# BVE-Reborn/rend3

Measured on AMD Instinct MI355X. Metric: shaded Mpixels/s @4K (whole frame: cull+compact all cameras, 4 shadow views, PBR opaque, tonemap), higher is better.
Workload: dtype f32; 1 GPU; BASELINE.json configs[2] stand-in: bistro_like (seed 0xB157, every object owns its geometry), 3840x2160, full PBR opaque + 4 directional shadow views (2048^2), camera dolly, 130 materials with base colour + normal + AO/roughness/metallic maps (RGBA8, mips, trilinear); objects=3000, triangles=2823212, cameras=5, parallelism=single GPU

## Files before the change

rend3_amd/csrc/kernels_shade.h:

```cpp
#pragma once
#include <type_traits>

#include "device_math.h"
#include "texture.h"

#define R3N_TEX_OCC 5
#define R3N_MS_OCC 4

struct TriRecord;
struct ViewLights;
struct ShadeArgs {
    const unsigned long long *vis;
    uint32_t width, height, row_begin, row_end;
    const r3n_frame_uniforms496 *fu;
    const r3n_camera_header240 *hdr;
    const r3n_object128 *objects;
    const uint32_t *mesh;
    const r3n_baked128 *baked;
    const r3n_material208 *materials;
    uint32_t n_materials;
    const uint32_t *tri_base;
    const uint32_t *slot_table;
    uint32_t slot_table_size;
    const uint8_t *dir_buf;
// ... 1049 lines not shown
    } else {
        h[0] = hdr[i0];
        h[1] = two ? hdr[i0 + 1u] : make_ushort4(0, 0, 0, 0);
    }
    uchar4 o8[2];
#pragma unroll
    for (int k = 0; k < 2; ++k) {
        o8[k] = tonemap_half4(srgb_lut, h[k], bgr);
        if (out_f32 != nullptr && (k == 0 || two)) {
            const float r = (float)__builtin_bit_cast(_Float16, h[k].x), g = (float)__builtin_bit_cast(_Float16, h[k].y);
            const float b = (float)__builtin_bit_cast(_Float16, h[k].z), al = (float)__builtin_bit_cast(_Float16, h[k].w);
            out_f32[i0 + (size_t)k] = make_float4(manual ? srgb_scene_to_display(r) : srgb_oetf(r), manual ? srgb_scene_to_display(g) : srgb_oetf(g),
                                                  manual ? srgb_scene_to_display(b) : srgb_oetf(b),
                                                  (!(al > 0.0f)) ? 0.0f : (al >= 1.0f ? 1.0f : al));
        }
    }
    out[i0] = o8[0];
    if (two) out[i0 + 1u] = o8[1];
}
#endif

extern "C" {
int r3n_internal_build_srgb_lut(unsigned char *lut, hipStream_t stream);
int r3n_internal_shade_prepass(const ShadeArgs *a, int tex, size_t first_key, size_t n_keys, hipStream_t stream);
int r3n_internal_resolve(const ShadeArgs *a, uint32_t samples, int tex, int rec, int split, int fast, hipStream_t stream);
int r3n_internal_resolve_class(const ShadeArgs *a, uint32_t variant, int fast, hipStream_t stream);
int r3n_internal_blend_apply(const ShadeArgs *a, const BlendApplyArgs *b, uint32_t samples, int tex, hipStream_t stream);
int r3n_internal_resolve_samples(const ushort4 *samples, ushort4 *hdr_out, size_t first_pixel, size_t n_pixels, hipStream_t stream);
int r3n_internal_tonemap(const ushort4 *hdr, uchar4 *out, float4 *out_f32, size_t first_pixel, size_t n_pixels, const unsigned char *srgb_lut,
                         uint32_t output_format, hipStream_t stream);
}
```

rend3_amd/csrc/r3n.hip:

```cpp
#include <fcntl.h>
#include <hip/hip_runtime.h>
#include <time.h>
#include <unistd.h>

#include <algorithm>
#include <atomic>
#include <cstdio>
#include <cstdlib>
#include <cstring>
#include <map>
#include <string>
#include <vector>

#include "comm.h"
#include "kernels_cull.h"
#include "kernels_raster.h"
#define R3N_SHADE_DECL_ONLY
#include "kernels_shade.h"
#include "skybox.h"
#include "blend_sort.h"
#include "morph.h"

namespace {

// ... 43 lines not shown
#define R3N_QLANES R3N_AUX_STREAMS
static_assert(R3N_AUX_STREAMS >= 1, "the shadow views draw on auxiliary streams");

struct r3n_ctx {
    int device = 0;
    hipStream_t stream = nullptr;
    hipStream_t aux[R3N_AUX_STREAMS] = {};
    hipEvent_t fork_ev[R3N_AUX_STREAMS] = {};
    hipStream_t shade = nullptr;
    hipEvent_t vp_ev = nullptr, shade_done[2] = {nullptr, nullptr};
    bool shade_pending[2] = {false, false};
    bool shade_unjoined = false;
    int shade_last = 0;
    int slot = 0;
    uint64_t frame_no = 0;
    bool overlap = true;
    bool always_fork = false;
    bool resolve_classes = true;
    bool fused_frame = false;
    DevBuf alt_vis, alt_atlas, alt_vp_baked;
    static constexpr size_t kFbUniforms = 0, kFbViewportHdr = 512, kFbDir = 768, kFbShadowHdr = 3072,
                            kFbPoint = kFbShadowHdr + 256 * R3N_MAX_SHADOW_VIEWS, kFbBytes = kFbPoint + 8448;
    static constexpr int kFbHost = 4;
    DevBuf fb_dev[2];
    uint8_t *fb_host[kFbHost] = {};
    hipEvent_t fb_ev[kFbHost] = {};
    bool fb_pending[kFbHost] = {};
    uint64_t main_epoch = 1, lane_epoch[R3N_AUX_STREAMS] = {};
    DevBuf big_count_all;
    std::vector<uint8_t> h_dir, h_point;
    uint64_t lights_version = 1, slot_lights_version[2] = {0, 0};
    hipEvent_t join_ev[R3N_AUX_STREAMS] = {};
    bool aux_used[R3N_AUX_STREAMS] = {};
    bool multi_stream = true;
    std::string err;
    DevBuf mesh, objects, materials, material_keys, dir_buf, point_buf, fu;
    DevBuf spheres, obj_meta;
    bool meta_dirty = false;
    uint32_t capacity = 0, n_materials = 0;
    std::vector<uint32_t> h_ntri;
    std::vector<uint32_t> h_material;
    std::vector<uint8_t> h_material_key;
    std::vector<r3n_material208> h_materials;
    std::vector<uint8_t> h_tex_short;
    DevBuf material_feat;
    DevBuf view_lights[2];
    uint32_t resolve_variants = 0;
    bool classes_dirty = true;
    struct Tune {
        uint32_t big_lds = R3N_BIG_LDS, vp_big_lds = R3N_VIEWPORT_BIG_LDS;
        uint32_t small_lds = R3N_SMALL_LDS, vp_small_lds = 0;
        uint32_t cut_big_lds = 0, vp_cut_big_lds = 0, cut_small_lds = 0, vp_cut_small_lds = 0;
        uint32_t prio_main = 1, prio_shade = 1, prio_aux = 1;
        uint32_t timed_pipeline = 0;
// ... 3 lines not shown
        uint32_t comm_serial = 1;
    } tune;
    bool cutout_short_dirty = true, cutout_short = false;
    bool key_census_dirty = true;
    uint64_t key_objects[3] = {0, 0, 0};
    uint64_t total_tris = 0;
    bool tri_base_dirty = true;
    DevBuf tri_base, slot_table;
    DevBuf skin_inputs, skin_matrices, skin_wave_skeleton, skin_wave_first, skin_joint_counts;
    uint32_t skinning_mode = R3N_SKIN_EXACT, skin_max_joints = 0;
    std::vector<r3n_skinning_input40> h_skin_inputs;
    uint32_t skin_total_waves = 0;
    DevBuf morph_block;
    uint32_t slot_table_size = 0;
    CamState canon;
    uint32_t width = 0, height = 0, samples = 1, atlas_w = 0, atlas_h = 0;
    float clear[4] = {0, 0, 0, 0};
    bool in_frame = false;
    bool blended_this_frame = false;
    bool resolved_this_frame = false;
    DevBuf vis, hdr16, out8, out_f32, atlas, hiz;
    r3n_hiz_desc hizd{};
    bool hiz_plane_ready = false;
    DevBuf tri_rec, tri_seen;
    DevBuf blend_order, blend_rank_base, frag_keys, frag_vals, frag_count, frag_head, samples16;
    uint32_t *status_host = nullptr, *status_dev = nullptr;
    std::vector<uint32_t> h_blend_order;
    uint32_t n_blend = 0, blend_tris = 0;
    DevBuf blend_set_slots, blend_set_locations, blend_sort_scratch;
    bool blend_sorted = false;
    uint32_t frag_capacity = 32u << 20;
    DevBuf tex_descs, tex_texels, tex_level_off, srgb8_decode;
    uint32_t n_textures = 0;
    uint64_t n_texels = 0;
    struct Cube { size_t first_word; uint32_t n, srgb; };
    DevBuf cube_texels;
    std::vector<Cube> cubes;
    uint32_t sky_cube = 0;
    bool sky_window = false;
    bool resolve_on_shade = false;
    uint32_t sky_samples_form = R3N_SKY_SAMPLES_ALL;
    DevBuf edge_list, edge_count;
    uint32_t edge_capacity_override = 0;
    DevBuf anim_rigs, anim_joints, anim_clips, anim_tracks, anim_times, anim_values, pose_requests;
    std::vector<r3n_anim_rig16> h_anim_rigs;
    std::vector<r3n_anim_clip16> h_anim_clips;
    uint32_t n_pose_requests = 0, pose_matrix_end = 0, anim_max_joints = 1;
// ... 188 lines not shown
    }
    ~Timed() {
        if (c->sync_stages) {
            (void)hipStreamSynchronize(stream);
            crumb(c, "stage done", stage);
        }
        if (!a) return;
        (void)hipEventRecord(b, stream);
        c->spans.push_back({a, b, stage, stream});
    }
};

int cam_lane(const r3n_ctx *c, r3n_camera cam) {
    if (cam == R3N_CAMERA_VIEWPORT || !c->multi_stream) return 0;
    return 1 + (int)(cam % R3N_AUX_STREAMS);
}
hipStream_t lane_stream(const r3n_ctx *c, int lane) { return lane == 0 ? c->stream : c->aux[lane - 1]; }

int fork_lane(r3n_ctx *c, int lane) {
    if (lane == 0) return R3N_OK;
    const int k = lane - 1;
    c->aux_used[k] = true;
    if (c->lane_epoch[k] == c->main_epoch && !c->always_fork) return R3N_OK;
    HIP_TRY(c, hipEventRecord(c->fork_ev[k], c->stream));
    HIP_TRY(c, hipStreamWaitEvent(c->aux[k], c->fork_ev[k], 0));
    c->lane_epoch[k] = c->main_epoch;
    return R3N_OK;
}
int join_lanes(r3n_ctx *c) {
    for (int k = 0; k < R3N_AUX_STREAMS; ++k)
        if (c->aux_used[k]) {
            HIP_TRY(c, hipEventRecord(c->join_ev[k], c->aux[k]));
            HIP_TRY(c, hipStreamWaitEvent(c->stream, c->join_ev[k], 0));
            c->aux_used[k] = false;
        }
    return R3N_OK;
}
int join_shade(r3n_ctx *c) {
    if (c->shade_unjoined) {
        HIP_TRY(c, hipStreamWaitEvent(c->stream, c->shade_done[c->shade_last], 0));
        c->shade_unjoined = false;
    }
    return R3N_OK;
}
int sync_all(r3n_ctx *c) {
    crumb(c, "sync_all");
    int r = join_lanes(c);
    if (r != R3N_OK) return r;
    r = join_shade(c);
// ... 304 lines not shown
        g_create_error = "host-mapped status word allocation failed";
        r3n_destroy(c);
        return nullptr;
    }
    c->status_host[0] = 0u;
    if (const char *eb = std::getenv("R3N_BREADCRUMBS")) {
        static std::atomic<int> n_ctx{0};
        const std::string path = std::string(eb) + ".pid" + std::to_string((long long)getpid()) + ".ctx" + std::to_string(n_ctx.fetch_add(1));
        c->crumb_fd = open(path.c_str(), O_CREAT | O_WRONLY | O_APPEND, 0644);
        crumb(c, "created");
    }
    if (const char *es = std::getenv("R3N_SYNC_STAGES")) c->sync_stages = es[0] == '1';
    if (const char *e1 = std::getenv("R3N_SINGLE_STREAM")) c->multi_stream = !(e1[0] == '1');
    if (const char *e2 = std::getenv("R3N_PIPELINE")) c->overlap = !(e2[0] == '0');
    if (const char *e5 = std::getenv("R3N_RESOLVE_CLASSES")) c->resolve_classes = !(e5[0] == '0');
    if (const char *e6 = std::getenv("R3N_ALWAYS_FORK")) c->always_fork = e6[0] == '1';
    if (const char *e3 = std::getenv("R3N_EDGE_CAPACITY")) c->edge_capacity_override = (uint32_t)std::strtoul(e3, nullptr, 10);
    if (const char *e7 = std::getenv("R3N_BIG_CAPACITY"))
        if (const uint32_t n = (uint32_t)std::strtoul(e7, nullptr, 10)) c->big_capacity = n;
    if (const char *e8 = std::getenv("R3N_FRAG_CAPACITY"))
        if (const uint32_t n = (uint32_t)std::strtoul(e8, nullptr, 10)) c->frag_capacity = n;
    if (hipStreamCreateWithPriority(&c->shade, hipStreamNonBlocking, (int)c->tune.prio_shade - 1) != hipSuccess ||
        hipEventCreateWithFlags(&c->vp_ev, hipEventDisableTiming) != hipSuccess ||
        hipEventCreateWithFlags(&c->shade_done[0], hipEventDisableTiming) != hipSuccess ||
        hipEventCreateWithFlags(&c->shade_done[1], hipEventDisableTiming) != hipSuccess) {
        g_create_error = "shade stream creation failed";
        r3n_destroy(c);
        return nullptr;
    }
    for (int k = 0; k < R3N_AUX_STREAMS; ++k)
        if (hipStreamCreateWithPriority(&c->aux[k], hipStreamNonBlocking, (int)c->tune.prio_aux - 1) != hipSuccess ||
            hipEventCreateWithFlags(&c->fork_ev[k], hipEventDisableTiming) != hipSuccess ||
            hipEventCreateWithFlags(&c->join_ev[k], hipEventDisableTiming) != hipSuccess) {
            g_create_error = "auxiliary stream creation failed";
            r3n_destroy(c);
            return nullptr;
        }
    {
        hipStream_t order[2 + R3N_AUX_STREAMS] = {c->stream, c->shade};
        for (int k = 0; k < R3N_AUX_STREAMS; ++k) order[2 + k] = c->aux[k];
        void *probe = nullptr;
        if (hipMalloc(&probe, 256) == hipSuccess) {
            for (hipStream_t st : order) {
                (void)hipMemsetAsync(probe, 0, 256, st);
                (void)hipStreamSynchronize(st);
            }
            (void)hipFree(probe);
        }
    }
    bool ok = ensure(c, c->srgb_lut, R3N_SRGB_LUT_SIZE, false, -1) == R3N_OK && ensure(c, c->srgb8_decode, 512 * 4, false, -1) == R3N_OK &&
              ensure(c, c->tex_descs, sizeof(r3n_texture_desc32), false, 0) == R3N_OK && ensure(c, c->tex_texels, 4, false, 0) == R3N_OK && ensure(c, c->tex_level_off, 64, false, 0) == R3N_OK &&
              ensure(c, c->material_keys, 256, false, 0) == R3N_OK && ensure(c, c->materials, sizeof(r3n_material208), false, 0) == R3N_OK;
    for (int k = 0; ok && k < 2; ++k) ok = ensure(c, c->fb_dev[k], r3n_ctx::kFbBytes, false, 0) == R3N_OK;
    for (int k = 0; ok && k < r3n_ctx::kFbHost; ++k)
        ok = hipHostMalloc((void **)&c->fb_host[k], r3n_ctx::kFbBytes, hipHostMallocDefault) == hipSuccess &&
             hipEventCreateWithFlags(&c->fb_ev[k], hipEventDisableTiming) == hipSuccess;
    if (ok) {
        for (int k = 0; k < r3n_ctx::kFbHost; ++k) std::memset(c->fb_host[k], 0, r3n_ctx::kFbBytes);
        c->fu.p = c->fb_dev[0].as<uint8_t>() + r3n_ctx::kFbUniforms; c->fu.bytes = 512;
        c->dir_buf.p = c->fb_dev[0].as<uint8_t>() + r3n_ctx::kFbDir; c->dir_buf.bytes = r3n_ctx::kFbShadowHdr - r3n_ctx::kFbDir;
        c->point_buf.p = c->fb_dev[0].as<uint8_t>() + r3n_ctx::kFbPoint; c->point_buf.bytes = 8448;
    }
    ok = ok && ensure(c, c->big_count_all, (size_t)(1 + R3N_QLANES) * 64 * R3N_BIGQ * 4, false, 0) == R3N_OK;
    for (int lane = 0; ok && lane < 1 + R3N_QLANES; ++lane) {
        c->big_count[lane].p = c->big_count_all.as<uint32_t>() + (size_t)lane * 64 * R3N_BIGQ;
        c->big_count[lane].bytes = 64 * R3N_BIGQ * 4;
        ok = ensure(c, c->big_items[lane], (size_t)c->big_capacity * R3N_BIGQ * sizeof(r3n_big_item), false, -1) == R3N_OK &&
             ensure(c, c->big_uv[lane], (size_t)c->big_capacity * R3N_BIGQ * sizeof(r3n_big_uv), false, -1) == R3N_OK;
    }
    if (ok) {
        (void)r3n_internal_build_srgb_lut(c->srgb_lut.as<unsigned char>(), c->stream);
        float decode[512];
        for (int i = 0; i < 256; ++i) {
            const float e = (float)i / 255.0f;
            decode[i] = e;
            decode[256 + i] = e > 0.04045f ? std::pow((e + 0.055f) / 1.055f, 2.4f) : e / 12.92f;
// ... 23 lines not shown
        g_create_error = c->err;
        r3n_destroy(c);
        return nullptr;
    }
    return c;
}

void r3n_destroy(r3n_ctx *c) {
    if (!c) return;
    crumb(c, "destroy");
    (void)hipSetDevice(c->device);
    (void)r3n_comm_destroy(c);
    if (c->stream) (void)hipStreamSynchronize(c->stream);
    if (c->shade) (void)hipStreamSynchronize(c->shade);
    for (int k = 0; k < R3N_AUX_STREAMS; ++k)
        if (c->aux[k]) (void)hipStreamSynchronize(c->aux[k]);
    for (int lane = 0; lane < 1 + R3N_QLANES; ++lane)
        for (DevBuf *b : {&c->big_items[lane], &c->big_uv[lane]})
            if (b->p) (void)hipFree(b->p);
    for (int k = 0; k < r3n_ctx::kFbHost; ++k) {
        if (c->fb_host[k]) (void)hipHostFree(c->fb_host[k]);
        if (c->fb_ev[k]) (void)hipEventDestroy(c->fb_ev[k]);
    }
    DevBuf *bufs[] = {&c->mesh, &c->objects, &c->spheres, &c->obj_meta, &c->materials, &c->material_keys, &c->fb_dev[0], &c->fb_dev[1], &c->big_count_all, &c->owners,
                      &c->tri_base, &c->slot_table, &c->skin_inputs, &c->skin_matrices, &c->skin_wave_skeleton,
                      &c->skin_wave_first, &c->skin_joint_counts, &c->morph_block, &c->vis, &c->hdr16, &c->out8, &c->out_f32, &c->atlas, &c->hiz, &c->alt_vis, &c->alt_atlas, &c->alt_vp_baked, &c->srgb_lut, &c->srgb_thr, &c->tex_descs, &c->tex_texels, &c->tex_level_off, &c->srgb8_decode,
                      &c->tri_rec, &c->tri_seen, &c->blend_order, &c->blend_rank_base, &c->frag_keys, &c->frag_vals, &c->frag_head,
                      &c->frag_count, &c->samples16, &c->anim_rigs, &c->anim_joints, &c->anim_clips, &c->anim_tracks,
                      &c->anim_times, &c->anim_values, &c->pose_requests, &c->edge_list, &c->edge_count, &c->material_feat, &c->view_lights[0],
                      &c->view_lights[1], &c->cube_texels, &c->blend_set_slots, &c->blend_set_locations, &c->blend_sort_scratch};
    for (DevBuf *b : bufs)
        if (b->p) (void)hipFree(b->p);
    free_cam(c->canon);
    free_cam(c->viewport);
    for (auto &kv : c->shadows) free_cam(kv.second);
    if (c->vp_ev) (void)hipEventDestroy(c->vp_ev);
    for (auto e : c->shade_done)
        if (e) (void)hipEventDestroy(e);
    if (c->shade) (void)hipStreamDestroy(c->shade);
    for (auto &s : c->spans) { (void)hipEventDestroy(s.a); (void)hipEventDestroy(s.b); }
    for (auto e : c->event_pool) (void)hipEventDestroy(e);
    for (int k = 0; k < R3N_AUX_STREAMS; ++k) {
        if (c->fork_ev[k]) (void)hipEventDestroy(c->fork_ev[k]);
        if (c->join_ev[k]) (void)hipEventDestroy(c->join_ev[k]);
        if (c->aux[k]) (void)hipStreamDestroy(c->aux[k]);
    }
    if (c->stage) (void)hipHostFree(c->stage);
    if (c->status_host) (void)hipHostFree(c->status_host);
    for (auto &b : c->bulk) {
        if (b.p) (void)hipHostFree(b.p);
        if (b.ev) (void)hipEventDestroy(b.ev);
    }
    for (auto e : c->stage_half_done)
        if (e) (void)hipEventDestroy(e);
    if (c->stream) (void)hipStreamDestroy(c->stream);
    delete c;
}

const char *r3n_last_error(const r3n_ctx *c) { return c ? c->err.c_str() : g_create_error.c_str(); }
// ... 286 lines not shown
    };
    const std::vector<uint8_t> old_dir = c->h_dir, old_point = c->h_point;
    TRY(take(c->h_dir, dir, dir_bytes, 128, R3N_MAX_DIR_LIGHTS));
    TRY(take(c->h_point, point, point_bytes, 32, R3N_MAX_POINT_LIGHTS));
    if (old_dir != c->h_dir || old_point != c->h_point) ++c->lights_version;
    return R3N_OK;
}

static int frame_begin_impl(r3n_ctx *c, const r3n_frame_uniforms496 *u, uint32_t w, uint32_t h, uint32_t samples,
                            const float clear_color[4], uint32_t atlas_w, uint32_t atlas_h, const r3n_frame_desc *d) {
    if (!c || !u || !clear_color || !w || !h) return fail(c, R3N_ERR_INVALID_ARG, "frame_begin: bad args");
    if (samples != 1 && samples != 4) return fail(c, R3N_ERR_INVALID_ARG, "frame_begin: samples must be 1 or 4 (SampleCount::One | Four)");
    if (w > 65535 || h > 65535) return fail(c, R3N_ERR_UNSUPPORTED, "frame_begin: target larger than 65535");
    if ((uint64_t)w * h * samples >= (1ull << 29) || (uint64_t)atlas_w * atlas_h >= (1ull << 30) || atlas_w > 65535 || atlas_h > 65535)
        return fail(c, R3N_ERR_UNSUPPORTED, "frame_begin: target of 2^29 samples or more / shadow atlas of 2^30 texels or more");
    HIP_TRY(c, hipSetDevice(c->device));
    c->width = w; c->height = h; c->samples = samples; c->atlas_w = atlas_w; c->atlas_h = atlas_h;
    std::memcpy(c->clear, clear_color, 16);
    const int hs = (int)(c->frame_no % (uint64_t)r3n_ctx::kFbHost);
    c->slot = (int)(c->frame_no++ & 1u);
    std::swap(c->vis, c->alt_vis);
    std::swap(c->atlas, c->alt_atlas);
    std::swap(c->viewport.baked, c->alt_vp_baked);
    uint8_t *dev = c->fb_dev[c->slot].as<uint8_t>();
    c->fu.p = dev + r3n_ctx::kFbUniforms;
    c->dir_buf.p = dev + r3n_ctx::kFbDir;
    c->point_buf.p = dev + r3n_ctx::kFbPoint;
    c->viewport.d_hdr.p = dev + r3n_ctx::kFbViewportHdr; c->viewport.d_hdr.bytes = 256;
    for (auto &kv : c->shadows) { kv.second.d_hdr.p = dev + r3n_ctx::kFbShadowHdr + 256u * (size_t)kv.first; kv.second.d_hdr.bytes = 256; }
    if (c->shade_pending[c->slot]) {
        HIP_TRY(c, hipStreamWaitEvent(c->stream, c->shade_done[c->slot], 0));
        c->shade_pending[c->slot] = false;
    }
    if (c->fb_pending[hs]) {
        HIP_WAIT(c, hipEventSynchronize(c->fb_ev[hs]));
        c->fb_pending[hs] = false;
    }
    uint8_t *host = c->fb_host[hs];
    std::memcpy(host + r3n_ctx::kFbUniforms, u, sizeof *u);
    if (c->h_dir.size() < 16) c->h_dir.assign(16, 0);
    if (c->h_point.size() < 16) c->h_point.assign(16, 0);
    std::memcpy(host + r3n_ctx::kFbDir, c->h_dir.data(), c->h_dir.size());
    size_t upto = r3n_ctx::kFbShadowHdr;
    if (d) {
        std::memcpy(host + r3n_ctx::kFbViewportHdr, d->viewport_header, sizeof(r3n_camera_header240));
        for (uint32_t v = 0; v < d->n_shadow_views; ++v)
            std::memcpy(host + r3n_ctx::kFbShadowHdr + 256u * (size_t)v, &d->shadow_views[v].header, sizeof(r3n_camera_header240));
        upto += 256u * (size_t)d->n_shadow_views;
    }
    HIP_TRY(c, hipMemcpyAsync(dev, host, upto, hipMemcpyHostToDevice, c->stream));
    if (c->slot_lights_version[c->slot] != c->lights_version) {
        std::memcpy(host + r3n_ctx::kFbPoint, c->h_point.data(), c->h_point.size());
        HIP_TRY(c, hipMemcpyAsync(dev + r3n_ctx::kFbPoint, host + r3n_ctx::kFbPoint, c->h_point.size(), hipMemcpyHostToDevice, c->stream));
        c->slot_lights_version[c->slot] = c->lights_version;
    }
    HIP_TRY(c, hipEventRecord(c->fb_ev[hs], c->stream));
    c->fb_pending[hs] = true;
    const size_t npix = (size_t)w * h;
    TRY(ensure(c, c->vis, npix * samples * 8, false, -1));
    TRY(ensure(c, c->hdr16, npix * 8, false, -1));
    TRY(ensure(c, c->out8, npix * 4, false, -1));
    build_hiz_desc(c->hizd, w, h);
    TRY(ensure(c, c->hiz, hiz_elements(c->hizd) * 4, false, -1));
    const size_t apix = (size_t)std::max(1u, atlas_w) * std::max(1u, atlas_h);
    TRY(ensure(c, c->atlas, apix * 4, false, -1));
    {
        Timed t(c, R3N_STAGE_CLEAR);
        hipLaunchKernelGGL(k_frame_clear, dim3(2048), dim3(256), 0, c->stream, c->vis.as<uint32_t>(), npix * samples * 2, c->atlas.as<uint32_t>(), apix,
                           c->big_count_all.as<uint32_t>(), c->big_count_all.bytes / 4);
        TRY(check_launch(c, "k_frame_clear"));
    }
    ++c->main_epoch;
    TRY(refresh_obj_meta(c));
    TRY(refresh_tri_base(c));
    c->in_frame = true;
    for (auto &f : c->forward_index_lane) f = 0;
    c->resolved_this_frame = false;
    c->blended_this_frame = false;
    c->sky_window = false;
    c->hiz_plane_ready = false;
    c->viewport.culled = false;
    for (auto &kv : c->shadows) kv.second.culled = false;
    return R3N_OK;
}

int r3n_frame_begin(r3n_ctx *c, const r3n_frame_uniforms496 *u, uint32_t w, uint32_t h, uint32_t samples,
                    const float clear_color[4], uint32_t atlas_w, uint32_t atlas_h) {
    return frame_begin_impl(c, u, w, h, samples, clear_color, atlas_w, atlas_h, nullptr);
}

int r3n_skinning(r3n_ctx *c, const r3n_skinning_input40 *inputs, uint32_t n, const float *joint_matrices, uint32_t n_joints) {
    if (!c) return R3N_ERR_INVALID_ARG;
    if (n == 0) return R3N_OK;
    if (!inputs || n_joints == 0) return fail(c, R3N_ERR_INVALID_ARG, "skinning: null inputs");
    if (!joint_matrices && c->n_pose_requests == 0) return fail(c, R3N_ERR_INVALID_ARG, "skinning: no joint matrices and no queued poses");
// ... 225 lines not shown
    TRY(ensure(c, c->pose_requests, std::max<size_t>(n, 1) * sizeof *requests, false, -1));
    if (n) {
        TRY(upload_bulk(c, c->pose_requests.p, requests, (size_t)n * sizeof *requests));
    }
    c->n_pose_requests = n;
    c->pose_matrix_end = end;
    return R3N_OK;
}


int r3n_uniform_bake(r3n_ctx *c, r3n_camera cam, const r3n_camera_header240 *hdr) {
    if (!c || !hdr) return fail(c, R3N_ERR_INVALID_ARG, "uniform_bake: null");
    CamState *s = find_cam(c, cam, true);
    if (!s) return fail(c, R3N_ERR_INVALID_ARG, "uniform_bake: bad camera");
    if (hdr->object_count != c->capacity) return fail(c, R3N_ERR_INVALID_ARG, "uniform_bake: header.object_count != object capacity");
    if ((cam == R3N_CAMERA_VIEWPORT) != (hdr->shadow_index == R3N_INVALID) || (cam != R3N_CAMERA_VIEWPORT && hdr->shadow_index != cam))
        return fail(c, R3N_ERR_INVALID_ARG, "uniform_bake: header.shadow_index does not match camera");
    HIP_TRY(c, hipSetDevice(c->device));
    s->hdr = *hdr;
    s->has_hdr = true;
    s->baked_frame = c->frame_no;
    if (c->capacity == 0) return R3N_OK;
    TRY(refresh_obj_meta(c));
    s->d_hdr.p = c->fb_dev[c->slot].as<uint8_t>() + (cam == R3N_CAMERA_VIEWPORT ? r3n_ctx::kFbViewportHdr : r3n_ctx::kFbShadowHdr + 256u * (size_t)cam);
    s->d_hdr.bytes = 256;
    if (s->hdr_frame != c->frame_no) TRY(upload_small(c, s->d_hdr.p, hdr, sizeof *hdr));
    TRY(ensure(c, s->baked, (size_t)c->capacity * sizeof(r3n_baked128), true, 0));
    const int lane = cam_lane(c, cam);
    if (c->fused_frame && c->in_frame && chained_pass_fits(c)) {
        TRY(ensure(c, s->chain, (size_t)R3N_CHAINED_OBJECT_PASS_MAX_BLOCKS * sizeof(ObjChainRec), false, 0));
        TRY(ensure(c, s->vis_flags, c->capacity, true, 0));
        TRY(ensure(c, s->vis_list, (size_t)(c->capacity + 1u) * sizeof(r3n_vis_entry), false, -1));
        TRY(ensure(c, s->slot_base[s->cur], (size_t)c->capacity * 4u, true, 0xFF));
        TRY(ensure(c, s->sub_counts[s->cur], sizeof(r3n_sub_counts), false, 0));
        TRY(ensure(c, s->counts[s->cur], sizeof(r3n_cull_counts), false, 0));
        TRY(ensure(c, s->first_entry, first_entry_bytes(c), false, -1));
        TRY(fork_lane(c, lane));
        TRY(run_bake_and_object_pass(c, *s, s->cur, camera_own(c, *s), lane_stream(c, lane), cam == R3N_CAMERA_VIEWPORT));
        s->object_pass_frame = c->frame_no;
        return R3N_OK;
    }
    TRY(fork_lane(c, lane));
    hipStream_t stream = lane_stream(c, lane);
    Timed t(c, R3N_STAGE_BAKE, stream);
    const uint32_t threads = c->capacity * 4u;
    hipLaunchKernelGGL(k_uniform_bake, dim3((threads + 255u) / 256u), dim3(256), 0, stream,
                       s->d_hdr.as<r3n_camera_header240>(), c->objects.as<r3n_object128>(), s->baked.as<r3n_baked128>());
    return check_launch(c, "k_uniform_bake");
}

static void key_census(r3n_ctx *c) {
    if (!c->key_census_dirty) return;
    c->key_objects[0] = c->key_objects[1] = c->key_objects[2] = 0;
    for (uint32_t o = 0; o < c->capacity; ++o)
        if (c->h_ntri[o]) {
            const uint32_t mi = c->h_material[o];
            c->key_objects[mi < c->h_material_key.size() ? std::min<uint32_t>(c->h_material_key[mi], 2) : 0]++;
        }
    c->key_census_dirty = false;
}
// ... 12 lines not shown
    for (int k = 0; k < 3; ++k) s->key_objects[cur][k] = c->key_objects[k];
    const int lane = cam_lane(c, cam);
    hipStream_t stream = lane_stream(c, lane);
    {
        const uint32_t cap0 = c->capacity, nblocks0 = (cap0 + 255u) / 256u;
        TRY(ensure(c, s->vis_flags, cap0, true, 0));
        TRY(ensure(c, s->vis_list, (size_t)(cap0 + 1u) * sizeof(r3n_vis_entry), false, -1));
        TRY(ensure(c, s->block_sums, (size_t)nblocks0 * sizeof(ObjBlockSums), false, -1));
        TRY(ensure(c, s->block_off, (size_t)nblocks0 * sizeof(ObjBlockOffsets), false, -1));
        TRY(ensure(c, s->slot_base[cur], (size_t)cap0 * 4u, true, 0xFF));
        if (viewport && s->has_prev) TRY(ensure(c, s->slot_base[prev], (size_t)cap0 * 4u, true, 0xFF));
        TRY(ensure(c, s->sub_counts[cur], sizeof(r3n_sub_counts), false, 0));
        TRY(ensure(c, s->counts[cur], sizeof(r3n_cull_counts), false, 0));
        TRY(ensure(c, s->first_entry, first_entry_bytes(c), false, -1));
    }
    const uint32_t mw = max_waves(c);
    const uint32_t chunks = (mw + R3N_CHUNK_WAVES - 1u) / R3N_CHUNK_WAVES;
    const uint32_t subcap = ((chunks + R3N_SUBQ - 1u) / R3N_SUBQ) * (R3N_CHUNK_WAVES * 64u);
    const size_t list_bytes = (size_t)3 * R3N_SUBQ * subcap * sizeof(r3n_tri_ref);
    s->subcap[cur] = subcap;
    TRY(ensure(c, s->mask[cur], (size_t)mw * 8u, false, -1));
    TRY(ensure(c, s->predicted[cur], list_bytes, false, -1));
    if (viewport) TRY(ensure(c, s->residual, list_bytes, false, -1));
    TRY(fork_lane(c, lane));
    if (s->object_pass_frame != c->frame_no)
        TRY(run_object_pass(c, *s, cur, camera_own(c, *s), nullptr, stream));
    TriCullArgs a{};
    a.hdr = s->d_hdr.as<r3n_camera_header240>();
    a.objects = c->objects.as<r3n_object128>();
    a.mesh = c->mesh.as<uint32_t>();
    a.baked = s->baked.as<r3n_baked128>();
    a.material_keys = c->material_keys.as<uint8_t>();
    a.n_materials = c->n_materials;
    a.vis_list = s->vis_list.as<r3n_vis_entry>();
    a.first_entry = s->first_entry.as<uint32_t>();
    a.counts = s->counts[cur].as<r3n_cull_counts>();
    a.prev_slot_base = (viewport && s->has_prev) ? s->slot_base[prev].as<uint32_t>() : nullptr;
    a.prev_mask = (viewport && s->has_prev) ? s->mask[prev].as<unsigned long long>() : nullptr;
    a.mask = s->mask[cur].as<unsigned long long>();
    a.predicted = s->predicted[cur].as<r3n_tri_ref>();
    a.residual = viewport ? s->residual.as<r3n_tri_ref>() : nullptr;
    a.sub_counts = s->sub_counts[cur].as<r3n_sub_counts>();
    a.subcap = subcap;
    a.hiz.data = c->hiz.as<float>();
    a.hiz.d = c->hizd;
    const uint32_t grid = std::max(1u, std::min(chunks, 4096u));
    {
        Timed t(c, R3N_STAGE_TRIANGLE_CULL, stream);
        hipLaunchKernelGGL(k_triangle_cull, dim3(grid), dim3(256), viewport ? c->tune.vp_cull_lds : c->tune.cull_lds, stream, a);
// ... 218 lines not shown
    a.material_feat = nullptr;
    a.variants = 0u;
    return a;
}

int r3n_resolve_opaque(r3n_ctx *c) {
    if (!c || !c->in_frame) return fail(c, R3N_ERR_STATE, "resolve_opaque: outside a frame");
    HIP_TRY(c, hipSetDevice(c->device));
    const uint32_t r0 = std::min(c->row_begin, c->height), r1 = std::min(c->row_end, c->height);
    c->sky_window = r1 <= r0;
    c->resolve_on_shade = false;
    if (r1 <= r0) return R3N_OK;
    CamState &s = c->viewport;
    if (!s.has_hdr && c->capacity) return fail(c, R3N_ERR_STATE, "resolve_opaque: viewport uniforms not baked");
    const bool use_records = c->total_tris > 0 && (uint64_t)c->total_tris * sizeof(TriRecord) <= (8ull << 30);
    const uint64_t npix_all = (uint64_t)c->width * c->height;
    const bool blend_samples = c->samples == 4 && c->blend_tris > 0;
    const bool split = c->samples == 4 && use_records && !blend_samples && npix_all < (1ull << 29);
    uint32_t edge_cap = 0;
    const bool classes = use_records && c->samples == 1 && c->n_textures > 0 && c->n_materials > 0 && c->resolve_classes;
    if (classes) TRY(refresh_material_classes(c));
    if (use_records && c->samples == 1) TRY(ensure(c, c->view_lights[c->slot], sizeof(ViewLights), false, -1));
    if (use_records) {
        TRY(ensure(c, c->tri_rec, (size_t)c->total_tris * sizeof(TriRecord), false, -1));
        TRY(ensure(c, c->tri_seen, (size_t)c->total_tris, false, 0));
    }
    const bool sky = c->sky_cube != 0u;
    const bool sky_samples = sky && c->samples == 4 && !split && !blend_samples;
    if (blend_samples || split || sky_samples) TRY(ensure(c, c->samples16, (size_t)npix_all * 4 * 8, false, -1));
    if (split) {
        edge_cap = (uint32_t)((uint64_t)(r1 - r0) * c->width * 3u / R3N_EDGEQ) + 4096u;
        if (c->edge_capacity_override) edge_cap = c->edge_capacity_override;
        TRY(ensure(c, c->edge_list, (size_t)edge_cap * R3N_EDGEQ * 4, false, -1));
        TRY(ensure(c, c->edge_count, R3N_EDGEQ * 4, false, 0));
    }
    const bool on_shade = c->overlap && c->multi_stream && (!c->timing || c->tune.timed_pipeline != 0u) && c->blend_tris == 0;
    hipStream_t stream = on_shade ? c->shade : c->stream;
    if (on_shade) {
        HIP_TRY(c, hipEventRecord(c->vp_ev, c->stream));
        HIP_TRY(c, hipStreamWaitEvent(c->shade, c->vp_ev, 0));
        for (int k = 0; k < R3N_AUX_STREAMS; ++k)
            if (c->aux_used[k]) {
                HIP_TRY(c, hipEventRecord(c->join_ev[k], c->aux[k]));
                HIP_TRY(c, hipStreamWaitEvent(c->shade, c->join_ev[k], 0));
            }
    } else {
        TRY(join_lanes(c));
        TRY(join_shade(c));
    }
    ShadeArgs a = make_shade_args(c, r0, r1);
    if (blend_samples || sky_samples) a.samples_out = c->samples16.as<ushort4>();
    if (use_records && c->samples == 1) a.view_lights = c->view_lights[c->slot].as<ViewLights>();
    if (classes && c->resolve_variants != 0u) {
        a.material_feat = c->material_feat.as<uint32_t>();
        a.variants = c->resolve_variants;
    }
    c->resolved_this_frame = true;
    const bool tex = c->n_textures > 0;
    if (use_records) {
        a.tri_rec = c->tri_rec.as<TriRecord>();
        a.seen = c->tri_seen.as<unsigned char>();
        Timed t(c, R3N_STAGE_VERTEX, stream);
        const size_t first = (size_t)r0 * c->width * c->samples, npx = (size_t)(r1 - r0) * c->width * c->samples;
        HIP_TRY(c, (hipError_t)r3n_internal_shade_prepass(&a, tex ? 1 : 0, first, npx, stream));
    }
    {
        Timed t(c, R3N_STAGE_SHADE, stream);
        if (split) {
            a.samples_out = c->samples16.as<ushort4>();
            a.edge_list = c->edge_list.as<uint32_t>();
            a.edge_count = c->edge_count.as<uint32_t>();
            a.edge_capacity = edge_cap;
            HIP_TRY(c, hipMemsetAsync(a.edge_count, 0, R3N_EDGEQ * 4, stream));
        }
        HIP_TRY(c, (hipError_t)r3n_internal_resolve(&a, c->samples, tex ? 1 : 0, a.tri_rec != nullptr ? 1 : 0, split ? (sky ? 2 : 1) : 0,
                                                    c->shade_mode == R3N_SHADE_FAST ? 1 : 0, stream));
    }
    TRY(check_launch(c, "k_resolve_opaque"));
    if (on_shade) {
        HIP_TRY(c, hipEventRecord(c->shade_done[c->slot], c->shade));
        c->shade_pending[c->slot] = true;
        c->shade_unjoined = true;
        c->shade_last = c->slot;
    }
    c->sky_window = true;
    c->resolve_on_shade = on_shade;
    c->sky_samples_form = split ? R3N_SKY_SAMPLES_EDGES : R3N_SKY_SAMPLES_ALL;
    return R3N_OK;
// ... 561 lines not shown
    }
    return r3n_output_work_enqueued(c);
}

int r3n_render_frame(r3n_ctx *c, const r3n_frame_desc *d) {
    if (!c || !d || d->struct_size < sizeof(r3n_frame_desc)) return fail(c, R3N_ERR_INVALID_ARG, "render_frame: bad descriptor");
    if (!d->uniforms || !d->viewport_header || (d->n_shadow_views && !d->shadow_views) || d->n_shadow_views > R3N_MAX_SHADOW_VIEWS)
        return fail(c, R3N_ERR_INVALID_ARG, "render_frame: null uniforms / headers, or too many shadow views");
    if (c->in_frame) return fail(c, R3N_ERR_STATE, "render_frame: a frame is already open");
    const bool native = c->comm.on;
    crumb(c, "render_frame", d->width, d->height);
    if (native) {
        if (d->exchange) return fail(c, R3N_ERR_INVALID_ARG, "render_frame: an exchange callback AND r3n_comm_init communicators");
        band_rows(d->height, c->comm.world, c->comm.rank, c->row_begin, c->row_end);
    }
    for (uint32_t v = 0; v < d->n_shadow_views; ++v)
        if (d->shadow_views[v].header.shadow_index != v) return fail(c, R3N_ERR_INVALID_ARG, "render_frame: shadow view i must carry shadow_index i");
    if (d->directional_buffer) TRY(r3n_lights_write(c, d->directional_buffer, d->directional_bytes, d->point_buffer, d->point_bytes));
    TRY(frame_begin_impl(c, d->uniforms, d->width, d->height, d->samples, d->clear_color, d->shadow_atlas_width, d->shadow_atlas_height, d));
    c->viewport.hdr_frame = c->frame_no;
    for (uint32_t v = 0; v < d->n_shadow_views; ++v)
        if (CamState *s = find_cam(c, v, true)) {
            s->hdr_frame = c->frame_no;
            s->d_hdr.p = c->fb_dev[c->slot].as<uint8_t>() + r3n_ctx::kFbShadowHdr + 256u * (size_t)v;
            s->d_hdr.bytes = 256;
        }
    struct Closer {
        r3n_ctx *c; bool armed = true;
        ~Closer() { if (armed && c->in_frame) { const std::string keep = c->err; (void)close_frame(c); c->err = keep; } }
    } closer{c};
    struct Fused { r3n_ctx *c; ~Fused() { c->fused_frame = false; } } fused{c};
    c->fused_frame = true;
    const bool masked = native || (d->flags & R3N_FRAME_SHADOW_MASK) != 0u;
    auto mine = [&](uint32_t v) {
        if (native) return shadow_part_of(c->comm.world, d->n_shadow_views, c->comm.rank, v) >= 0;
        return !masked || ((d->shadow_view_mask >> v) & 1ull) != 0ull;
    };
    for (uint32_t v = 0; v < d->n_shadow_views; ++v) {
        const r3n_shadow_view272 &sv = d->shadow_views[v];
        TRY(r3n_shadow_viewport(c, v, sv.x, sv.y, sv.size));
        {
            CamState *s = find_cam(c, v, true);
            if (!s) return fail(c, R3N_ERR_INVALID_ARG, "render_frame: bad shadow camera");
            s->band_begin = 0; s->band_end = 0xFFFFFFFFu;
            const int part = native ? shadow_part_of(c->comm.world, d->n_shadow_views, c->comm.rank, v) : -1;
            if (part >= 0) band_rows(sv.size, shadow_parts(c->comm.world, d->n_shadow_views), (uint32_t)part, s->band_begin, s->band_end);
        }
// ... 479 lines not shown
```

rend3_amd/csrc/shade.hip:

```cpp
#include <hip/hip_runtime.h>

#include "kernels_shade.h"

namespace {
int launch_status() { return (int)hipGetLastError(); }
}

extern "C" int r3n_internal_resolve_ms(const ShadeArgs *ap, int tex, int rec, int split, hipStream_t stream);

extern "C" {

int r3n_internal_build_srgb_lut(unsigned char *lut, hipStream_t stream) {
    hipLaunchKernelGGL(k_build_srgb_lut, dim3((R3N_SRGB_LUT_SIZE + 255u) / 256u), dim3(256), 0, stream, lut);
    return launch_status();
}

int r3n_internal_shade_prepass(const ShadeArgs *ap, int tex, size_t first_key, size_t n_keys, hipStream_t stream) {
    const ShadeArgs &a = *ap;
    hipLaunchKernelGGL(k_mark_visible, dim3((unsigned)((n_keys + 255) / 256)), dim3(256), 0, stream, a.vis, a.seen, first_key, n_keys);
    const dim3 vgrid((unsigned)(((size_t)a.total_tris + 255) / 256));
    if (tex) hipLaunchKernelGGL(k_vertex_stage<true>, vgrid, dim3(256), 0, stream, a);
    else hipLaunchKernelGGL(k_vertex_stage<false>, vgrid, dim3(256), 0, stream, a);
    return launch_status();
}

int r3n_internal_resolve(const ShadeArgs *ap, uint32_t samples, int tex, int rec, int split, int fast, hipStream_t stream) {
    if (samples == 4) return r3n_internal_resolve_ms(ap, tex, rec, split, stream);
    const ShadeArgs &a = *ap;
    const dim3 rgrid((a.width + 15u) / 16u, (a.row_end - a.row_begin + 15u) / 16u);
    if (rec) {
        if (!a.view_lights) return (int)hipErrorInvalidValue;
        hipLaunchKernelGGL(k_stage_view_lights, dim3(1), dim3(256), 0, stream, a, const_cast<ViewLights *>(a.view_lights));
    }
    if (rec && tex && a.variants != 0u) {
        for (uint32_t v = 0; v < R3N_VARIANTS; ++v) {
            if (!((a.variants >> v) & 1u)) continue;
            if (v < R3N_VARIANTS - 1u) {
                const int rc = r3n_internal_resolve_class(ap, v, fast, stream);
                if (rc) return rc;
            } else if (fast) {
                hipLaunchKernelGGL((k_resolve_opaque<1, true, true, false, true>), rgrid, dim3(256), a.resolve_lds, stream, a);
            } else {
                hipLaunchKernelGGL((k_resolve_opaque<1, true, true>), rgrid, dim3(256), a.resolve_lds, stream, a);
            }
        }
    } else if (rec && fast) {
        if (tex) hipLaunchKernelGGL((k_resolve_opaque<1, true, true, false, true>), rgrid, dim3(256), a.resolve_lds, stream, a);
        else hipLaunchKernelGGL((k_resolve_opaque<1, false, true, false, true>), rgrid, dim3(256), a.resolve_lds, stream, a);
    } else if (rec) {
        if (tex) hipLaunchKernelGGL((k_resolve_opaque<1, true, true>), rgrid, dim3(256), a.resolve_lds, stream, a);
        else hipLaunchKernelGGL((k_resolve_opaque<1, false, true>), rgrid, dim3(256), a.resolve_lds, stream, a);
    } else {
        if (tex) hipLaunchKernelGGL((k_resolve_opaque<1, true, false>), rgrid, dim3(256), a.resolve_lds, stream, a);
        else hipLaunchKernelGGL((k_resolve_opaque<1, false, false>), rgrid, dim3(256), a.resolve_lds, stream, a);
    }
    return launch_status();
// ... 12 lines not shown
```

Before: 9612 Mpixels/s.

## Fork aux lanes early after frame upload and move shade prepass onto main stream

Aux camera lanes can now start their bake/object pass as soon as the per-frame constants upload finishes, rather than waiting on a fork event recorded later on the main stream. The constants blocks are quad-buffered and the triangle-record buffer double-buffered, and the wait on the previous frame's shade completion is moved after the upload. The vertex prepass and view-light staging now run on the main stream before the handoff to the shade stream. The aim is to cut cross-stream serialisation so culling of the next frame overlaps more with shading, at the cost of more memory and more intricate epoch-based fork logic that could introduce ordering hazards.

```diff
diff --git a/rend3_amd/csrc/kernels_shade.h b/rend3_amd/csrc/kernels_shade.h
--- a/rend3_amd/csrc/kernels_shade.h
+++ b/rend3_amd/csrc/kernels_shade.h
@@ -1095,7 +1095,7 @@
 
 extern "C" {
 int r3n_internal_build_srgb_lut(unsigned char *lut, hipStream_t stream);
-int r3n_internal_shade_prepass(const ShadeArgs *a, int tex, size_t first_key, size_t n_keys, hipStream_t stream);
+int r3n_internal_shade_prepass(const ShadeArgs *a, int tex, int lights, size_t first_key, size_t n_keys, hipStream_t stream);
 int r3n_internal_resolve(const ShadeArgs *a, uint32_t samples, int tex, int rec, int split, int fast, hipStream_t stream);
 int r3n_internal_resolve_class(const ShadeArgs *a, uint32_t variant, int fast, hipStream_t stream);
 int r3n_internal_blend_apply(const ShadeArgs *a, const BlendApplyArgs *b, uint32_t samples, int tex, hipStream_t stream);
diff --git a/rend3_amd/csrc/r3n.hip b/rend3_amd/csrc/r3n.hip
--- a/rend3_amd/csrc/r3n.hip
+++ b/rend3_amd/csrc/r3n.hip
@@ -89,14 +89,18 @@
     static constexpr size_t kFbUniforms = 0, kFbViewportHdr = 512, kFbDir = 768, kFbShadowHdr = 3072,
                             kFbPoint = kFbShadowHdr + 256 * R3N_MAX_SHADOW_VIEWS, kFbBytes = kFbPoint + 8448;
     static constexpr int kFbHost = 4;
-    DevBuf fb_dev[2];
+    DevBuf fb_dev[kFbHost];
+    int fb_slot = 0;
+    hipEvent_t head_ev = nullptr;
+    uint64_t upload_epoch = 0, clear_epoch = 0;
+    uint64_t lane_early_frame[R3N_AUX_STREAMS] = {};
     uint8_t *fb_host[kFbHost] = {};
     hipEvent_t fb_ev[kFbHost] = {};
     bool fb_pending[kFbHost] = {};
     uint64_t main_epoch = 1, lane_epoch[R3N_AUX_STREAMS] = {};
     DevBuf big_count_all;
     std::vector<uint8_t> h_dir, h_point;
-    uint64_t lights_version = 1, slot_lights_version[2] = {0, 0};
+    uint64_t lights_version = 1, slot_lights_version[kFbHost] = {};
     hipEvent_t join_ev[R3N_AUX_STREAMS] = {};
     bool aux_used[R3N_AUX_STREAMS] = {};
     bool multi_stream = true;
@@ -146,7 +150,7 @@
     DevBuf vis, hdr16, out8, out_f32, atlas, hiz;
     r3n_hiz_desc hizd{};
     bool hiz_plane_ready = false;
-    DevBuf tri_rec, tri_seen;
+    DevBuf tri_rec[2], tri_seen;
     DevBuf blend_order, blend_rank_base, frag_keys, frag_vals, frag_count, frag_head, samples16;
     uint32_t *status_host = nullptr, *status_dev = nullptr;
     std::vector<uint32_t> h_blend_order;
@@ -381,9 +385,24 @@
     const int k = lane - 1;
     c->aux_used[k] = true;
     if (c->lane_epoch[k] == c->main_epoch && !c->always_fork) return R3N_OK;
-    HIP_TRY(c, hipEventRecord(c->fork_ev[k], c->stream));
-    HIP_TRY(c, hipStreamWaitEvent(c->aux[k], c->fork_ev[k], 0));
+    if (c->lane_early_frame[k] == c->frame_no && c->main_epoch == c->clear_epoch && !c->always_fork) {
+        HIP_TRY(c, hipStreamWaitEvent(c->aux[k], c->head_ev, 0));
+    } else {
+        HIP_TRY(c, hipEventRecord(c->fork_ev[k], c->stream));
+        HIP_TRY(c, hipStreamWaitEvent(c->aux[k], c->fork_ev[k], 0));
+    }
     c->lane_epoch[k] = c->main_epoch;
+    return R3N_OK;
+}
+int fork_lane_early(r3n_ctx *c, int lane) {
+    if (lane == 0) return R3N_OK;
+    const int k = lane - 1;
+    const bool head = c->fused_frame && !c->always_fork && c->main_epoch == c->clear_epoch && c->clear_epoch == c->upload_epoch + 1u;
+    if (!head || c->lane_epoch[k] == c->main_epoch) return fork_lane(c, lane);
+    c->aux_used[k] = true;
+    if (c->lane_early_frame[k] == c->frame_no) return R3N_OK;
+    HIP_TRY(c, hipStreamWaitEvent(c->aux[k], c->fb_ev[c->fb_slot], 0));
+    c->lane_early_frame[k] = c->frame_no;
     return R3N_OK;
 }
 int join_lanes(r3n_ctx *c) {
@@ -734,6 +753,7 @@
         if (const uint32_t n = (uint32_t)std::strtoul(e8, nullptr, 10)) c->frag_capacity = n;
     if (hipStreamCreateWithPriority(&c->shade, hipStreamNonBlocking, (int)c->tune.prio_shade - 1) != hipSuccess ||
         hipEventCreateWithFlags(&c->vp_ev, hipEventDisableTiming) != hipSuccess ||
+        hipEventCreateWithFlags(&c->head_ev, hipEventDisableTiming) != hipSuccess ||
         hipEventCreateWithFlags(&c->shade_done[0], hipEventDisableTiming) != hipSuccess ||
         hipEventCreateWithFlags(&c->shade_done[1], hipEventDisableTiming) != hipSuccess) {
         g_create_error = "shade stream creation failed";
@@ -763,7 +783,7 @@
     bool ok = ensure(c, c->srgb_lut, R3N_SRGB_LUT_SIZE, false, -1) == R3N_OK && ensure(c, c->srgb8_decode, 512 * 4, false, -1) == R3N_OK &&
               ensure(c, c->tex_descs, sizeof(r3n_texture_desc32), false, 0) == R3N_OK && ensure(c, c->tex_texels, 4, false, 0) == R3N_OK && ensure(c, c->tex_level_off, 64, false, 0) == R3N_OK &&
               ensure(c, c->material_keys, 256, false, 0) == R3N_OK && ensure(c, c->materials, sizeof(r3n_material208), false, 0) == R3N_OK;
-    for (int k = 0; ok && k < 2; ++k) ok = ensure(c, c->fb_dev[k], r3n_ctx::kFbBytes, false, 0) == R3N_OK;
+    for (int k = 0; ok && k < r3n_ctx::kFbHost; ++k) ok = ensure(c, c->fb_dev[k], r3n_ctx::kFbBytes, false, 0) == R3N_OK;
     for (int k = 0; ok && k < r3n_ctx::kFbHost; ++k)
         ok = hipHostMalloc((void **)&c->fb_host[k], r3n_ctx::kFbBytes, hipHostMallocDefault) == hipSuccess &&
              hipEventCreateWithFlags(&c->fb_ev[k], hipEventDisableTiming) == hipSuccess;
@@ -833,10 +853,11 @@
         if (c->fb_host[k]) (void)hipHostFree(c->fb_host[k]);
         if (c->fb_ev[k]) (void)hipEventDestroy(c->fb_ev[k]);
     }
-    DevBuf *bufs[] = {&c->mesh, &c->objects, &c->spheres, &c->obj_meta, &c->materials, &c->material_keys, &c->fb_dev[0], &c->fb_dev[1], &c->big_count_all, &c->owners,
+    static_assert(r3n_ctx::kFbHost == 4, "the list below names every constants block");
+    DevBuf *bufs[] = {&c->mesh, &c->objects, &c->spheres, &c->obj_meta, &c->materials, &c->material_keys, &c->fb_dev[0], &c->fb_dev[1], &c->fb_dev[2], &c->fb_dev[3], &c->big_count_all, &c->owners,
                       &c->tri_base, &c->slot_table, &c->skin_inputs, &c->skin_matrices, &c->skin_wave_skeleton,
                       &c->skin_wave_first, &c->skin_joint_counts, &c->morph_block, &c->vis, &c->hdr16, &c->out8, &c->out_f32, &c->atlas, &c->hiz, &c->alt_vis, &c->alt_atlas, &c->alt_vp_baked, &c->srgb_lut, &c->srgb_thr, &c->tex_descs, &c->tex_texels, &c->tex_level_off, &c->srgb8_decode,
-                      &c->tri_rec, &c->tri_seen, &c->blend_order, &c->blend_rank_base, &c->frag_keys, &c->frag_vals, &c->frag_head,
+                      &c->tri_rec[0], &c->tri_rec[1], &c->tri_seen, &c->blend_order, &c->blend_rank_base, &c->frag_keys, &c->frag_vals, &c->frag_head,
                       &c->frag_count, &c->samples16, &c->anim_rigs, &c->anim_joints, &c->anim_clips, &c->anim_tracks,
                       &c->anim_times, &c->anim_values, &c->pose_requests, &c->edge_list, &c->edge_count, &c->material_feat, &c->view_lights[0],
                       &c->view_lights[1], &c->cube_texels, &c->blend_set_slots, &c->blend_set_locations, &c->blend_sort_scratch};
@@ -846,6 +867,7 @@
     free_cam(c->viewport);
     for (auto &kv : c->shadows) free_cam(kv.second);
     if (c->vp_ev) (void)hipEventDestroy(c->vp_ev);
+    if (c->head_ev) (void)hipEventDestroy(c->head_ev);
     for (auto e : c->shade_done)
         if (e) (void)hipEventDestroy(e);
     if (c->shade) (void)hipStreamDestroy(c->shade);
@@ -1178,16 +1200,13 @@
     std::swap(c->vis, c->alt_vis);
     std::swap(c->atlas, c->alt_atlas);
     std::swap(c->viewport.baked, c->alt_vp_baked);
-    uint8_t *dev = c->fb_dev[c->slot].as<uint8_t>();
+    c->fb_slot = hs;
+    uint8_t *dev = c->fb_dev[hs].as<uint8_t>();
     c->fu.p = dev + r3n_ctx::kFbUniforms;
     c->dir_buf.p = dev + r3n_ctx::kFbDir;
     c->point_buf.p = dev + r3n_ctx::kFbPoint;
     c->viewport.d_hdr.p = dev + r3n_ctx::kFbViewportHdr; c->viewport.d_hdr.bytes = 256;
     for (auto &kv : c->shadows) { kv.second.d_hdr.p = dev + r3n_ctx::kFbShadowHdr + 256u * (size_t)kv.first; kv.second.d_hdr.bytes = 256; }
-    if (c->shade_pending[c->slot]) {
-        HIP_TRY(c, hipStreamWaitEvent(c->stream, c->shade_done[c->slot], 0));
-        c->shade_pending[c->slot] = false;
-    }
     if (c->fb_pending[hs]) {
         HIP_WAIT(c, hipEventSynchronize(c->fb_ev[hs]));
         c->fb_pending[hs] = false;
@@ -1204,14 +1223,19 @@
             std::memcpy(host + r3n_ctx::kFbShadowHdr + 256u * (size_t)v, &d->shadow_views[v].header, sizeof(r3n_camera_header240));
         upto += 256u * (size_t)d->n_shadow_views;
     }
+    c->upload_epoch = c->main_epoch;
     HIP_TRY(c, hipMemcpyAsync(dev, host, upto, hipMemcpyHostToDevice, c->stream));
-    if (c->slot_lights_version[c->slot] != c->lights_version) {
+    if (c->slot_lights_version[hs] != c->lights_version) {
         std::memcpy(host + r3n_ctx::kFbPoint, c->h_point.data(), c->h_point.size());
         HIP_TRY(c, hipMemcpyAsync(dev + r3n_ctx::kFbPoint, host + r3n_ctx::kFbPoint, c->h_point.size(), hipMemcpyHostToDevice, c->stream));
-        c->slot_lights_version[c->slot] = c->lights_version;
+        c->slot_lights_version[hs] = c->lights_version;
     }
     HIP_TRY(c, hipEventRecord(c->fb_ev[hs], c->stream));
     c->fb_pending[hs] = true;
+    if (c->shade_pending[c->slot]) {
+        HIP_TRY(c, hipStreamWaitEvent(c->stream, c->shade_done[c->slot], 0));
+        c->shade_pending[c->slot] = false;
+    }
     const size_t npix = (size_t)w * h;
     TRY(ensure(c, c->vis, npix * samples * 8, false, -1));
     TRY(ensure(c, c->hdr16, npix * 8, false, -1));
@@ -1226,7 +1250,8 @@
                            c->big_count_all.as<uint32_t>(), c->big_count_all.bytes / 4);
         TRY(check_launch(c, "k_frame_clear"));
     }
-    ++c->main_epoch;
+    c->clear_epoch = ++c->main_epoch;
+    if (d) HIP_TRY(c, hipEventRecord(c->head_ev, c->stream));
     TRY(refresh_obj_meta(c));
     TRY(refresh_tri_base(c));
     c->in_frame = true;
@@ -1498,7 +1523,7 @@
     s->baked_frame = c->frame_no;
     if (c->capacity == 0) return R3N_OK;
     TRY(refresh_obj_meta(c));
-    s->d_hdr.p = c->fb_dev[c->slot].as<uint8_t>() + (cam == R3N_CAMERA_VIEWPORT ? r3n_ctx::kFbViewportHdr : r3n_ctx::kFbShadowHdr + 256u * (size_t)cam);
+    s->d_hdr.p = c->fb_dev[c->fb_slot].as<uint8_t>() + (cam == R3N_CAMERA_VIEWPORT ? r3n_ctx::kFbViewportHdr : r3n_ctx::kFbShadowHdr + 256u * (size_t)cam);
     s->d_hdr.bytes = 256;
     if (s->hdr_frame != c->frame_no) TRY(upload_small(c, s->d_hdr.p, hdr, sizeof *hdr));
     TRY(ensure(c, s->baked, (size_t)c->capacity * sizeof(r3n_baked128), true, 0));
@@ -1511,7 +1536,7 @@
         TRY(ensure(c, s->sub_counts[s->cur], sizeof(r3n_sub_counts), false, 0));
         TRY(ensure(c, s->counts[s->cur], sizeof(r3n_cull_counts), false, 0));
         TRY(ensure(c, s->first_entry, first_entry_bytes(c), false, -1));
-        TRY(fork_lane(c, lane));
+        TRY(fork_lane_early(c, lane));
         TRY(run_bake_and_object_pass(c, *s, s->cur, camera_own(c, *s), lane_stream(c, lane), cam == R3N_CAMERA_VIEWPORT));
         s->object_pass_frame = c->frame_no;
         return R3N_OK;
@@ -1570,9 +1595,12 @@
     TRY(ensure(c, s->mask[cur], (size_t)mw * 8u, false, -1));
     TRY(ensure(c, s->predicted[cur], list_bytes, false, -1));
     if (viewport) TRY(ensure(c, s->residual, list_bytes, false, -1));
-    TRY(fork_lane(c, lane));
-    if (s->object_pass_frame != c->frame_no)
+    if (s->object_pass_frame == c->frame_no) {
+        TRY(fork_lane_early(c, lane));
+    } else {
+        TRY(fork_lane(c, lane));
         TRY(run_object_pass(c, *s, cur, camera_own(c, *s), nullptr, stream));
+    }
     TriCullArgs a{};
     a.hdr = s->d_hdr.as<r3n_camera_header240>();
     a.objects = c->objects.as<r3n_object128>();
@@ -1837,7 +1865,7 @@
     if (classes) TRY(refresh_material_classes(c));
     if (use_records && c->samples == 1) TRY(ensure(c, c->view_lights[c->slot], sizeof(ViewLights), false, -1));
     if (use_records) {
-        TRY(ensure(c, c->tri_rec, (size_t)c->total_tris * sizeof(TriRecord), false, -1));
+        TRY(ensure(c, c->tri_rec[c->slot], (size_t)c->total_tris * sizeof(TriRecord), false, -1));
         TRY(ensure(c, c->tri_seen, (size_t)c->total_tris, false, 0));
     }
     const bool sky = c->sky_cube != 0u;
@@ -1851,7 +1879,25 @@
     }
     const bool on_shade = c->overlap && c->multi_stream && (!c->timing || c->tune.timed_pipeline != 0u) && c->blend_tris == 0;
     hipStream_t stream = on_shade ? c->shade : c->stream;
+    ShadeArgs a = make_shade_args(c, r0, r1);
+    if (blend_samples || sky_samples) a.samples_out = c->samples16.as<ushort4>();
+    if (use_records && c->samples == 1) a.view_lights = c->view_lights[c->slot].as<ViewLights>();
+    if (classes && c->resolve_variants != 0u) {
+        a.material_feat = c->material_feat.as<uint32_t>();
+        a.variants = c->resolve_variants;
+    }
+    const bool tex = c->n_textures > 0;
+    auto prepass = [&]() -> int {
+        if (!use_records) return R3N_OK;
+        a.tri_rec = c->tri_rec[c->slot].as<TriRecord>();
+        a.seen = c->tri_seen.as<unsigned char>();
+        Timed t(c, R3N_STAGE_VERTEX, c->stream);
+        const size_t first = (size_t)r0 * c->width * c->samples, npx = (size_t)(r1 - r0) * c->width * c->samples;
+        HIP_TRY(c, (hipError_t)r3n_internal_shade_prepass(&a, tex ? 1 : 0, a.view_lights != nullptr ? 1 : 0, first, npx, c->stream));
+        return R3N_OK;
+    };
     if (on_shade) {
+        TRY(prepass());
         HIP_TRY(c, hipEventRecord(c->vp_ev, c->stream));
         HIP_TRY(c, hipStreamWaitEvent(c->shade, c->vp_ev, 0));
         for (int k = 0; k < R3N_AUX_STREAMS; ++k)
@@ -1862,23 +1908,9 @@
     } else {
         TRY(join_lanes(c));
         TRY(join_shade(c));
-    }
-    ShadeArgs a = make_shade_args(c, r0, r1);
-    if (blend_samples || sky_samples) a.samples_out = c->samples16.as<ushort4>();
-    if (use_records && c->samples == 1) a.view_lights = c->view_lights[c->slot].as<ViewLights>();
-    if (classes && c->resolve_variants != 0u) {
-        a.material_feat = c->material_feat.as<uint32_t>();
-        a.variants = c->resolve_variants;
+        TRY(prepass());
     }
     c->resolved_this_frame = true;
-    const bool tex = c->n_textures > 0;
-    if (use_records) {
-        a.tri_rec = c->tri_rec.as<TriRecord>();
-        a.seen = c->tri_seen.as<unsigned char>();
-        Timed t(c, R3N_STAGE_VERTEX, stream);
-        const size_t first = (size_t)r0 * c->width * c->samples, npx = (size_t)(r1 - r0) * c->width * c->samples;
-        HIP_TRY(c, (hipError_t)r3n_internal_shade_prepass(&a, tex ? 1 : 0, first, npx, stream));
-    }
     {
         Timed t(c, R3N_STAGE_SHADE, stream);
         if (split) {
@@ -2486,7 +2518,7 @@
     for (uint32_t v = 0; v < d->n_shadow_views; ++v)
         if (CamState *s = find_cam(c, v, true)) {
             s->hdr_frame = c->frame_no;
-            s->d_hdr.p = c->fb_dev[c->slot].as<uint8_t>() + r3n_ctx::kFbShadowHdr + 256u * (size_t)v;
+            s->d_hdr.p = c->fb_dev[c->fb_slot].as<uint8_t>() + r3n_ctx::kFbShadowHdr + 256u * (size_t)v;
             s->d_hdr.bytes = 256;
         }
     struct Closer {
diff --git a/rend3_amd/csrc/shade.hip b/rend3_amd/csrc/shade.hip
--- a/rend3_amd/csrc/shade.hip
+++ b/rend3_amd/csrc/shade.hip
@@ -15,12 +15,14 @@
     return launch_status();
 }
 
-int r3n_internal_shade_prepass(const ShadeArgs *ap, int tex, size_t first_key, size_t n_keys, hipStream_t stream) {
+int r3n_internal_shade_prepass(const ShadeArgs *ap, int tex, int lights, size_t first_key, size_t n_keys, hipStream_t stream) {
     const ShadeArgs &a = *ap;
+    if (lights && !a.view_lights) return (int)hipErrorInvalidValue;
     hipLaunchKernelGGL(k_mark_visible, dim3((unsigned)((n_keys + 255) / 256)), dim3(256), 0, stream, a.vis, a.seen, first_key, n_keys);
     const dim3 vgrid((unsigned)(((size_t)a.total_tris + 255) / 256));
     if (tex) hipLaunchKernelGGL(k_vertex_stage<true>, vgrid, dim3(256), 0, stream, a);
     else hipLaunchKernelGGL(k_vertex_stage<false>, vgrid, dim3(256), 0, stream, a);
+    if (lights) hipLaunchKernelGGL(k_stage_view_lights, dim3(1), dim3(256), 0, stream, a, const_cast<ViewLights *>(a.view_lights));
     return launch_status();
 }
 
@@ -28,10 +30,7 @@
     if (samples == 4) return r3n_internal_resolve_ms(ap, tex, rec, split, stream);
     const ShadeArgs &a = *ap;
     const dim3 rgrid((a.width + 15u) / 16u, (a.row_end - a.row_begin + 15u) / 16u);
-    if (rec) {
-        if (!a.view_lights) return (int)hipErrorInvalidValue;
-        hipLaunchKernelGGL(k_stage_view_lights, dim3(1), dim3(256), 0, stream, a, const_cast<ViewLights *>(a.view_lights));
-    }
+    if (rec && !a.view_lights) return (int)hipErrorInvalidValue;
     if (rec && tex && a.variants != 0u) {
         for (uint32_t v = 0; v < R3N_VARIANTS; ++v) {
             if (!((a.variants >> v) & 1u)) continue;
```

After: 9645 Mpixels/s, median of 2. About the same (+0.3%).
